# cipherflow-fhe/lattisense

Measured on AMD Instinct MI355X. Metric: ckks_hmult_relin_rescale_throughput, higher is better.
Workload: dtype u64

## Files before the change

lattisense_amd/csrc/emu_ntt.cpp:

```cpp
#define LSA_EMULATE 1
#include <cstddef>
#include <vector>
#include "ntt_plan.h"
#include "ntt_r16.h"
#include <array>
#include "tables.h"

template <int NT>
static void emu_block(const NttPassArgs& a, const NttBlockCtx& bc, u64* lds) {
    for (int t = 0; t < NT; t++) ntt_phase_load<true, NT>(a, bc, t, lds);
    int rho[4];
    const int np = ntt_split(a.mu, rho);
    if (!a.inverse) {
        int sig = 0;
        for (int i = 0; i < np; i++) {
            for (int t = 0; t < NT; t++) ntt_phase_sub_dyn<NT>(a, bc, t, lds, sig, rho[i]);
            sig += rho[i];
        }
    } else {
        int sig = a.mu;
        for (int i = np - 1; i >= 0; i--) {
            sig -= rho[i];
            for (int t = 0; t < NT; t++) ntt_phase_sub_dyn<NT>(a, bc, t, lds, sig, rho[i]);
        }
    }
    for (int t = 0; t < NT; t++) ntt_phase_store<true, NT>(a, bc, t, lds);
}

template <int PASS, int MU>
static void emu_block_r16(const NttPassArgs& a, const NttBlockCtx& bc, u64* lds) {
    std::vector<std::array<u64, 16>> regs(LSA_R16_THREADS);
    for (int phase = 0; phase < 3; phase++)
        for (int t = 0; t < LSA_R16_THREADS; t++) {
            u64(&v)[16] = *reinterpret_cast<u64(*)[16]>(regs[t].data());
            r16_phase<PASS, 3, MU>(a, bc, t, lds, phase, v);
        }
}

static void emu_block_r8x3(const NttPassArgs& a, const NttBlockCtx& bc, u64* lds) {
    std::vector<std::array<u64, 16>> regs(LSA_R16_THREADS);
    for (int phase = 0; phase < 4; phase++)
        for (int t = 0; t < LSA_R16_THREADS; t++) {
            u64(&v)[16] = *reinterpret_cast<u64(*)[16]>(regs[t].data());
            r8x3_phase<3>(a, bc, t, lds, phase, v);
        }
}

extern "C" int lsa_emu_ntt(int n, const u64* moduli, int nmod, u64* data, int batch, long long batch_stride, int rows,
                           const unsigned char* mod_of, int period, int inverse, int tau_max, int allow_fp64) {
    const int row_inner = (allow_fp64 >> 1) & 1;
    const bool r16 = (allow_fp64 >> 2) & 1;
    allow_fp64 &= 1;
    lsa::HostTables T;
    T.build(n, std::vector<u64>(moduli, moduli + nmod));
    NttPlan plan = make_ntt_plan(T.logn, tau_max);
    std::vector<u64> tw_i(T.psi.size());
    std::vector<double> tw_d(T.psi_d.size());
    for (int m = 0; m < nmod; m++) {
        const size_t o = (size_t)m * n;
        ntt_permute_twiddles(plan, T.logn, (inverse ? T.psiinv : T.psi).data() + 2 * o, tw_i.data() + 2 * o, 2, false);
        ntt_permute_twiddles(plan, T.logn, (inverse ? T.psiinv_d : T.psi_d).data() + o, tw_d.data() + o, 1, true);
    }
    NttPassArgs a{};
    a.src = data;
// ... 1 lines not shown
    a.src_stride = batch_stride;
    a.dst_stride = batch_stride;
    a.batch = batch;
    a.rows = rows;
    a.mods = T.mods.data();
    a.tw = tw_i.data();
    a.scale = T.scale.data();
    a.twd = tw_d.data();
    a.scaled = T.scale_d.data();
    a.allow_fp64 = allow_fp64;
    a.period = period;
    a.row0 = 0;
    a.row_step = 1;
    a.row_inner = row_inner;
    for (int i = 0; i < period; i++) a.mod_of[i] = mod_of[i];
    int launch_rows = 0;
    for (int r = 0; r < rows; r++)
        if (mod_of[r % period] != LSA_ROW_SKIP) a.row_tbl[launch_rows++] = (unsigned short)r;
    a.compact = 1;
    a.rows = launch_rows;
    for (int step = 0; step < plan.npass; step++) {
        int k = inverse ? plan.npass - 1 - step : step;
        ntt_fill_pass(a, plan, T.logn, k, inverse);
        a.fp_raw_out = plan.npass == 2 && step == 0;
        a.fp_raw_in = plan.npass == 2 && step == 1;
        std::vector<u64> lds(lds_words(a.tau));
        long long nblocks = (long long)batch * launch_rows * (1 << (a.logn - a.tau));
        for (long long bid = 0; bid < nblocks; bid++) {
            NttBlockCtx bc = ntt_decode_block(a, bid);
            if (bc.mod == LSA_ROW_SKIP) continue;
            if (r16 && ntt_r16_shape_ok(a, plan.npass)) {
                if (a.mu == 9) emu_block_r8x3(a, bc, lds.data());
                else if (a.lambda && a.mu == 8) emu_block_r16<0, 8>(a, bc, lds.data());
                else if (a.lambda) emu_block_r16<0, 7>(a, bc, lds.data());
                else if (a.mu == 8) emu_block_r16<1, 8>(a, bc, lds.data());
                else emu_block_r16<1, 7>(a, bc, lds.data());
            } else if (a.tau <= 12) emu_block<LSA_NTT_THREADS>(a, bc, lds.data());
            else if (a.tau == 13) emu_block<512>(a, bc, lds.data());
            else emu_block<1024>(a, bc, lds.data());
        }
    }
    return 0;
}
```

lattisense_amd/csrc/kernels.hip:

```cpp
#include <atomic>
#include <cstdlib>

#include "build_flags.h"
#include "lsa_internal.h"
#include "ntt_r16.h"

namespace lsa {

const char* kernels_build_flags() { return LSA_BUILD_FLAGS_TEXT; }

static constexpr int TPB = 256;

#ifndef LSA_NTT_WAVES
#define LSA_NTT_WAVES 4
#endif

#if defined(LSA_NTT_DIAG_STAMPS)
#define LSA_STAMP(k)                                                                               \
    do {                                                                                           \
        if (a.diag && threadIdx.x == 0 && blockIdx.x < 8192) a.diag[blockIdx.x * 8 + (k)] = __builtin_amdgcn_s_memtime(); \
    } while (0)
#else
#define LSA_STAMP(k) do { } while (0)
#endif
// ... 41 lines not shown
#if defined(LSA_NTT_STAGGER)
    {
        const int phase = blockIdx.x < 768 ? (int)(blockIdx.x >> 8) : 0;
        for (int i = 0; i < phase * LSA_NTT_STAGGER; i++) __builtin_amdgcn_s_sleep(100);
    }
#endif
#if defined(LSA_NTT_DIAG_COMPUTE_ONLY)
    for (int i = tid; i < (1 << a.tau); i += NT)
        lds[lds_addr(i)] = bc.fp ? d_to_bits((double)(i * 7 + 1)) : (u64)(i * 7 + 1);
    __syncthreads();
    ntt_butterfly_phases<NT>(a, bc, tid, lds);
    if (lds[lds_addr(tid)] == 0x123456789abcull) a.dst[bc.base_dst + tid] = 1;
    return;
#endif
    LSA_STAMP(0);
    ntt_phase_load<(FZ & 1) != 0, NT>(a, bc, tid, lds);
    if (TWL && tid < (1 << a.mu)) {
        u64* tw_l = lds + lds_words(a.tau);
        if (bc.fp) tw_l[tid] = twp.x;
        else {
            tw_l[2 * tid] = twp.x;
            tw_l[2 * tid + 1] = twp.y;
        }
    }
    LSA_STAMP(1);
    __syncthreads();
    LSA_STAMP(2);
#if defined(LSA_NTT_DIAG_COPY_ONLY)
    ntt_phase_store<(FZ & 2) != 0, NT, (FZ & 4) != 0, (FZ & 8) != 0>(a, bc, tid, lds);
    return;
#endif
// ... 42 lines not shown
    u64 v[16];
    r8x3_phase<FZ>(a, bc, tid, lds, 0, v);
    r16_sync<1>();
    r8x3_phase<FZ>(a, bc, tid, lds, 1, v);
    r16_sync<1>();
    r8x3_phase<FZ>(a, bc, tid, lds, 2, v);
    r16_sync<1>();
    r8x3_phase<FZ>(a, bc, tid, lds, 3, v);
}
static bool ntt_launch_r16(const NttPassArgs& a, int npass, bool fused, long long nblocks, hipStream_t s) {
    static const bool enabled = [] {
        const char* e = getenv("LSA_NTT_R16");
        return !(e && e[0] == '0');
    }();
    if (!enabled || !ntt_r16_shape_ok(a, npass)) return false;
    const bool pro = fused && a.fz_pro && a.s_lo == 0, epi = fused && a.fz_epi && a.final_reduce;
    const size_t lds_bytes = (size_t)LSA_R16_LDS_WORDS * sizeof(u64);
    const dim3 grid((unsigned)nblocks), block(LSA_R16_THREADS);
    if (epi && a.fz_epi == 3) {
        if (a.lambda) return false;
        if (a.mu == 9) {
            const char* e = getenv("LSA_NTT_R8X3");
            if (e && e[0] == '0') return false;
            hipLaunchKernelGGL((k_ntt_r8x3<4>), grid, block, lds_bytes, s, a);
        } else if (a.mu == 8) {
            hipLaunchKernelGGL((k_ntt_r16<1, 4, 8>), grid, block, lds_bytes, s, a);
        } else {
            hipLaunchKernelGGL((k_ntt_r16<1, 4, 7>), grid, block, lds_bytes, s, a);
        }
        LSA_HIP(hipGetLastError());
        return true;
    }
    if (epi && a.fz_epi == 4) {
// ... 73 lines not shown
    a.mu = MU;
    a.lambda = 0;
    a.tau = 12;
    a.inverse = 0;
    a.apply_scale = 0;
    a.final_reduce = 1;
    a.fp_raw_in = g.fp_raw_in;
    a.fp_raw_out = 0;
    a.mods = g.mods;
    a.tw = g.tw;
    a.twd = g.twd;
    a.scale = nullptr;
    a.scaled = nullptr;
    a.src = g.ext;
    a.fz_pro = a.fz_epi = 0;
    NttBlockCtx bc;
    bc.tile = tile;
    bc.mod = tl < g.L ? tl : g.nq + (tl - g.L);
    bc.fp = FP;
    bc.b = (int)b;
    bc.row = 0;
    bc.tw_l = nullptr;
    bc.base_dst = 0;
    const R16Limb L = r16_limb(a, bc);
    const int kj = tl < g.L ? tl : g.klvl + 1 + (tl - g.L);
    const int own_d = tl < g.L ? tl / g.np : -1;
    int k, i;
    r16_lane<1, MU>(tid, k, i);
    const unsigned G1 = r16_G1<1, MU>(bc, k), G2 = (G1 << 4) + ((unsigned)i << (MU <= 8 ? 8 - MU : 0));
    u64 acc0[16], acc1[16];
// ... 128 lines not shown
        int dev = 0;
        LSA_HIP(hipGetDevice(&dev));
        const unsigned long long bit = 1ull << (dev & 63);
        if (!(raised.load(std::memory_order_acquire) & bit)) {
            LSA_HIP(hipFuncSetAttribute(reinterpret_cast<const void*>(&k_ntt_pass<FZ, NT>), hipFuncAttributeMaxDynamicSharedMemorySize, 160 * 1024));
            raised.fetch_or(bit, std::memory_order_release);
        }
    }
    hipLaunchKernelGGL((k_ntt_pass<FZ, NT>), dim3((unsigned)nblocks), dim3(NT), lds_bytes, s, a);
    LSA_HIP(hipGetLastError());
}

template <int NT>
static void ntt_launch_pass(const NttPassArgs& a, bool fused, long long nblocks, size_t lds_bytes, hipStream_t s) {
    LSA_REQUIRE((1 << a.tau) <= 2 * LSA_NTT_STAGE_PAIRS * NT, "ntt: tile larger than the staging registers");
    const bool pro = fused && a.fz_pro && a.s_lo == 0, epi = fused && a.fz_epi && a.final_reduce;
    if (epi && a.fz_epi == 3) {
        ntt_launch_variant<4, NT>(a, nblocks, lds_bytes, s);
        return;
    }
    if (epi && a.fz_epi == 4) {
        ntt_launch_variant<8, NT>(a, nblocks, lds_bytes, s);
        return;
    }
    switch ((pro ? 1 : 0) | (epi ? 2 : 0)) {
        case 0: ntt_launch_variant<0, NT>(a, nblocks, lds_bytes, s); break;
        case 1: ntt_launch_variant<1, NT>(a, nblocks, lds_bytes, s); break;
        case 2: ntt_launch_variant<2, NT>(a, nblocks, lds_bytes, s); break;
        default: ntt_launch_variant<3, NT>(a, nblocks, lds_bytes, s); break;
    }
}
// ... 4 lines not shown
}

void launch_ntt(Context& c, const u64* src, u64* dst, int batch, long long src_stride, long long dst_stride, int rows,
                const RowMap& rm, bool inverse, hipStream_t s, const NttFusion* fz, int passes) {
    if (batch <= 0 || rows <= 0) return;
    LSA_REQUIRE(rm.period >= 1 && rm.period <= LSA_MAX_PERIOD, "ntt: bad row-map period");
    NttPassArgs a{};
    a.batch = batch;
    a.rows = rows;
    a.mods = c.d_mods;
    a.scale = c.d_scale;
    a.diag = c.ntt_diag;
    a.scaled = c.d_scale_d;
    a.allow_fp64 = c.fp64_ntt;
    if (fz) {
        LSA_REQUIRE(!inverse, "fused tails exist for forward transforms only");
        a.fz_epi = fz->epi;
        a.fz_pro = fz->pro;
        a.fz_limbs = fz->limbs;
        a.fz_base_polys = fz->base_polys;
        a.fz_ql_mod = fz->ql_mod;
        a.fz_a = fz->a;
        a.fz_a_stride = fz->a_stride;
        a.fz_a_rpp = fz->a_rpp;
        a.fz_base = fz->base;
        a.fz_base_stride = fz->base_stride;
        a.fz_base_rpp = fz->base_rpp;
        a.fz_k = fz->k;
        a.fz_out = fz->out;
        a.fz_out_stride = fz->out_stride;
        a.fz_out_rpp = fz->out_rpp;
        a.fz_last = fz->last;
        a.fz_last_stride = fz->last_stride;
        a.fz_last_rpp = fz->last_rpp;
        a.fz_k2 = fz->k2;
        a.fz_scatter = fz->scatter;
        LSA_REQUIRE(fz->epi != 2 || fz->k2, "merged tail needs its second factor");
        LSA_REQUIRE(!fz->scatter || fz->epi, "a scattered store needs an epilogue");
        LSA_REQUIRE(fz->epi != 3 || (!fz->pro && !fz->scatter && fz->a && fz->out), "pt_mul epilogue: plaintext and output, nothing else");
        LSA_REQUIRE(fz->epi != 4 || (!fz->pro && !fz->k2 && fz->scatter && fz->a && fz->k && fz->out && fz->pt),
                    "rotate-and-MAC epilogue: ModDown operands, index map, plaintext and output");
        LSA_REQUIRE(fz->epi != 4 || (fz->base_polys <= 1 && fz->limbs == rm.period), "rotate-and-MAC epilogue: base on poly 0, one row per limb");
        a.fz_pt = fz->pt;
        a.fz_pt_stride = fz->pt_stride;
        a.fz_accum = fz->accumulate ? 1 : 0;
    }
    a.period = rm.period;
    a.row0 = rm.row0;
    a.row_step = rm.row_step;
    for (int i = 0; i < rm.period; i++) {
        LSA_REQUIRE(rm.mod_of[i] == LSA_ROW_SKIP || rm.mod_of[i] < c.nmod, "ntt: modulus index out of range");
        a.mod_of[i] = rm.mod_of[i];
    }
    int active_rows = 0;
    for (int r = 0; r < rows; r++) active_rows += rm.mod_of[(rm.row0 + r * rm.row_step) % rm.period] != LSA_ROW_SKIP;
    if (active_rows == 0) return;
    int launch_rows = rows;
    a.compact = 0;
    if (active_rows <= LSA_MAX_PERIOD && rm.row0 + (rows - 1) * rm.row_step < 65536) {
        a.compact = 1;
// ... 4 lines not shown
        }
        launch_rows = active_rows;
    }
    a.rows = launch_rows;
    bool wide = c.plan_wide.npass < c.plan.npass && c.wide_mode != 0;
    if (wide && c.wide_mode == 2) {
        bool all_fp = c.fp64_ntt != 0;
        for (int r = 0; r < rows && all_fp; r++) {
            const unsigned char m = rm.mod_of[(rm.row0 + r * rm.row_step) % rm.period];
            if (m != LSA_ROW_SKIP && (c.T.mods[m].q >> LSA_FP64_MAX_BITS) != 0) all_fp = false;
        }
        const long long limbs = (long long)active_rows * batch;
        wide = !fz && (c.logn == 13 ? limbs >= 1024 : (all_fp && limbs >= 512));
    }
    if (passes != 3) wide = false;
    const NttPlan& plan = wide ? c.plan_wide : c.plan;
    a.tw = wide ? (inverse ? c.d_psiinv_w : c.d_psi_w) : (inverse ? c.d_psiinv : c.d_psi);
    a.twd = wide ? (inverse ? c.d_psiinv_d_w : c.d_psi_d_w) : (inverse ? c.d_psiinv_d : c.d_psi_d);
    {
        bool any_fp = false, any_int = false;
        for (int r = 0; r < rows; r++) {
            const unsigned char m = rm.mod_of[(rm.row0 + r * rm.row_step) % rm.period];
            if (m == LSA_ROW_SKIP) continue;
            const bool fp = c.fp_engine(m);
            any_fp |= fp;
            any_int |= !fp;
        }
        a.row_inner = any_fp && any_int;
    }
    int chunk = batch;
// ... 3 lines not shown
    }
    for (int b0 = 0; b0 < batch; b0 += chunk) {
        const int nb = std::min(chunk, batch - b0);
        a.batch = nb;
        if (fz && fz->epi == 3) {
            a.fz_a = fz->a + (long long)b0 * fz->a_stride;
            a.fz_base = fz->base ? fz->base + (long long)b0 * fz->base_stride : nullptr;
            a.fz_out = fz->out + (long long)b0 * fz->out_stride;
        }
        if (fz && fz->epi == 4) {
            a.fz_a = fz->a + (long long)b0 * fz->a_stride;
            a.fz_base = fz->base ? fz->base + (long long)b0 * fz->base_stride : nullptr;
            a.fz_pt = fz->pt + (long long)b0 * fz->pt_stride;
            a.fz_out = fz->out + (long long)b0 * fz->out_stride;
        }
        for (int step = 0; step < plan.npass; step++) {
            if (plan.npass == 2 && !((passes >> step) & 1)) continue;
            const int k = inverse ? plan.npass - 1 - step : step;
            ntt_fill_pass(a, plan, c.logn, k, inverse ? 1 : 0);
            a.fp_raw_out = plan.npass == 2 && step == 0 && c.fp_raw;
            a.fp_raw_in = plan.npass == 2 && step == 1 && c.fp_raw;
            a.src = (step == 0 ? src + (long long)b0 * src_stride : dst + (long long)b0 * dst_stride);
            a.src_stride = step == 0 ? src_stride : dst_stride;
            a.dst = dst + (long long)b0 * dst_stride;
            a.dst_stride = dst_stride;
            a.total_tiles = (long long)nb * launch_rows * (1 << (a.logn - a.tau));
            const long long nblocks = a.total_tiles;
            LSA_REQUIRE(nblocks < (1LL << 31), "ntt: grid too large");
            const size_t lds_bytes = (size_t)lds_words(a.tau) * sizeof(u64);
            ProfScope ps(c, PROF_NTT, 16.0 * c.n * active_rows * nb / plan.npass, s);
            if (ntt_launch_r16(a, plan.npass, fz != nullptr, nblocks, s)) continue;
            if (a.tau <= 12) ntt_launch_pass<LSA_NTT_THREADS>(a, fz != nullptr, nblocks, lds_bytes, s);
            else if (a.tau == 13) ntt_launch_pass<512>(a, fz != nullptr, nblocks, lds_bytes, s);
            else ntt_launch_pass<1024>(a, fz != nullptr, nblocks, lds_bytes, s);
        }
    }
}

struct EwArgs {
    const u64* a;
    const u64* b;
    const u64* acc;
    u64* out;
    long long sa, sb, so, sacc;
    const ModDev* mods;
// ... 400 lines not shown
    g.pb = (long long)(b_rpp ? b_rpp : limbs) << c.logn;
    g.a = a;
    g.b = b;
    g.d = d;
    g.sa = sa;
    g.sb = sb;
    g.sd = sd;
    g.mods = c.d_mods;
    g.limbs = limbs;
    g.logn = c.logn;
    LSA_REQUIRE(rm.period == limbs && limbs <= LSA_MAX_PERIOD, "tensor: row map must cover the limbs");
    int period;
    fill_rowmap(g.mod_of, period, rm, c.nmod);
    ProfScope ps(c, PROF_TENSOR, 7.0 * 8 * c.n * limbs * batch, s);
    hipLaunchKernelGGL(k_tensor, ew_grid(c, limbs, batch), dim3(TPB), 0, s, g);
    LSA_HIP(hipGetLastError());
}

__global__ __launch_bounds__(TPB) void k_tensor_d2(TensorArgs g) {
    const int chunks = (1 << g.logn) / (2 * TPB);
    const int limb = blockIdx.x / chunks;
    const int x = ((blockIdx.x % chunks) * TPB + threadIdx.x) * 2;
    const ModDev m = g.mods[limb];
    const long long b = blockIdx.y;
    const long long off = ((long long)limb << g.logn) + x;
    const ulonglong2 a1 = ld2(g.a + b * g.sa + g.pa + off), b1 = ld2(g.b + b * g.sb + g.pb + off);
    st2(g.d + b * g.sd + off, mont_mul(a1.x, mont_mul_lazy(b1.x, m.r2, m.q, m.qinv), m.q, m.qinv),
        mont_mul(a1.y, mont_mul_lazy(b1.y, m.r2, m.q, m.qinv), m.q, m.qinv));
}

void launch_tensor_d2(Context& c, const u64* a, const u64* b, u64* d2, int batch, long long sa, long long sb, long long sd,
                      int limbs, hipStream_t s, int a_rpp, int b_rpp) {
    if (batch <= 0) return;
    TensorArgs g{};
    LSA_REQUIRE((a_rpp == 0 || a_rpp >= limbs) && (b_rpp == 0 || b_rpp >= limbs), "tensor: rows per polynomial below the limb count");
    LSA_REQUIRE(limbs <= c.nq, "tensor: Q limbs only");
    g.pa = (long long)(a_rpp ? a_rpp : limbs) << c.logn;
    g.pb = (long long)(b_rpp ? b_rpp : limbs) << c.logn;
    g.a = a;
    g.b = b;
    g.d = d2;
    g.sa = sa;
    g.sb = sb;
    g.sd = sd;
    g.mods = c.d_mods;
    g.limbs = limbs;
    g.logn = c.logn;
    ProfScope ps(c, PROF_TENSOR, 3.0 * 8 * c.n * limbs * batch, s);
    hipLaunchKernelGGL(k_tensor_d2, ew_grid(c, limbs, batch), dim3(TPB), 0, s, g);
    LSA_HIP(hipGetLastError());
}

struct BaseConvArgs {
    const BaseConvConsts* k;
    const ModDev* mods;
    const u64* src;
    u64* dst;
    long long ssrc, sdst;
    int logn;
    BaseConvRows rows;
    const u64* sub;
    long long ssub;
    int sub_row[LSA_BC_MAX_SRC];
};
// ... 1188 lines not shown
```

lattisense_amd/csrc/lsa_internal.h:

```cpp
#pragma once
#include <hip/hip_runtime.h>
#include <cstdint>
#include <map>
#include <memory>
#include <mutex>
#include <stdexcept>
#include <string>
#include <vector>

#include "../../include/lattisense_amd.h"
#include "ntt_plan.h"
#include "tables.h"

namespace lsa {

struct Error : std::runtime_error {
    int code;
    Error(int c, const std::string& m) : std::runtime_error(m), code(c) {}
};

void set_last_error(const std::string& m);

#define LSA_HIP(expr)                                                                                     \
    do {                                                                                                  \
// ... 174 lines not shown
    const u64* base = nullptr;
    long long base_stride = 0;
    int base_rpp = 0;
    const u64* k = nullptr;
    u64* out = nullptr;
    long long out_stride = 0;
    int out_rpp = 0;
    const u64* last = nullptr;
    long long last_stride = 0;
    int last_rpp = 1;
    const u64* k2 = nullptr;
    const u32* scatter = nullptr;
    const u64* pt = nullptr;
    long long pt_stride = 0;
    bool accumulate = false;
};
void launch_ntt(Context& c, const u64* src, u64* dst, int batch, long long src_stride, long long dst_stride, int rows,
                const RowMap& rm, bool inverse, hipStream_t s, const NttFusion* fz = nullptr, int passes = 3);

enum EwOp { EW_ADD = 0, EW_SUB = 1, EW_NEG = 2, EW_MUL = 3 };
void launch_elementwise(Context& c, EwOp op, const u64* a, const u64* b, u64* out, int batch, long long sa,
                        long long sb, long long so, int rows, const RowMap& rm, hipStream_t s);
void launch_muladd(Context& c, EwOp op, const u64* a, const u64* b, const u64* acc, long long sacc, u64* out, int batch,
                   long long sa, long long sb, long long so, int rows, const RowMap& rm, hipStream_t s);
#define LSA_MAC_MAX_TERMS 16
#define LSA_MACM_MAX 8
void launch_mac_plain(Context& c, int terms, const u64* const* ct, const long long* sct, const u64* const* pt,
                      const long long* spt, const u64* partial, long long spartial, u64* out, long long so, int batch,
                      int polys, int limbs, const RowMap& rm, hipStream_t s);
void launch_mac_plain_multi(Context& c, int nb, const u64* const* ct, const long long* sct, int ng, const u64* const* pt,
                            u64* const* out, long long so, int batch, int polys, int limbs, const RowMap& rm, hipStream_t s);
void launch_mont_muladd(Context& c, const u64* a, long long sa, const u64* pt, long long spt, const u64* acc, long long sacc,
                        u64* out, long long so, int batch, int polys, int limbs, const RowMap& rm, hipStream_t s);
void launch_lift_ringt(Context& c, int mode, int level, const u64* pt, long long spt, u64* out, long long sout, int batch,
                       hipStream_t s);
void launch_tensor(Context& c, const u64* a, const u64* b, u64* d, int batch, long long sa, long long sb, long long sd,
                   int limbs, const RowMap& rm, hipStream_t s, int a_rpp = 0, int b_rpp = 0);
void launch_tensor_d2(Context& c, const u64* a, const u64* b, u64* d2, int batch, long long sa, long long sb, long long sd,
                      int limbs, hipStream_t s, int a_rpp = 0, int b_rpp = 0);
struct TensorFold {
    const u64* a;
    const u64* b;
    long long sa, sb;
    long long pa, pb;
};
struct BaseConvRows {
    int src_row[LSA_BC_MAX_SRC];
    int dst_row[LSA_BC_MAX_DST];
};
void launch_baseconv(Context& c, const BaseConvPlan* k, const BaseConvRows& rows, const u64* src, u64* dst, int batch,
                     long long ssrc, long long sdst, hipStream_t s, const u64* sub = nullptr, long long ssub = 0,
                     const int* sub_row = nullptr);
void launch_ks_mac(Context& c, int level, const u64* cx, long long scx, const u64* ext, long long sext,
                   const Key& key, u64* acc, long long sacc, int batch, hipStream_t s, bool unfused_only = false,
// ... 113 lines not shown
```

lattisense_amd/csrc/ntt_core.h:

```cpp
#pragma once
#include "modarith.h"

#ifndef LSA_NTT_THREADS
#define LSA_NTT_THREADS 256
#endif
#define LSA_MAX_PERIOD 192
#if defined(LSA_EMULATE)
#include <cstdio>
#include <cstdlib>
#define LSA_EMU_CHECK(c) do { if (!(c)) { std::fprintf(stderr, "ntt replay: range invariant violated: %s (%s:%d)\n", #c, __FILE__, __LINE__); std::abort(); } } while (0)
#else
#define LSA_EMU_CHECK(c) do { } while (0)
#endif
#define LSA_ROW_SKIP 0xFF
#define LSA_FP64_MAX_BITS 47
#ifndef LSA_NTT_MAX_RHO
#define LSA_NTT_MAX_RHO 4
#endif

struct NttPassArgs {
    const u64* src;
    u64* dst;
    long long src_stride;
    long long dst_stride;
// ... 19 lines not shown
    int fz_epi, fz_pro, fz_limbs, fz_base_polys, fz_ql_mod;
    int fz_a_rpp, fz_base_rpp, fz_out_rpp, fz_last_rpp;
    const u64* fz_a;
    const u64* fz_base;
    const u64* fz_k;
    const u64* fz_k2;
    u64* fz_out;
    const unsigned* fz_scatter;
    const u64* fz_last;
    long long fz_a_stride, fz_base_stride, fz_out_stride, fz_last_stride;
    unsigned long long* diag;
    unsigned char mod_of[LSA_MAX_PERIOD];
    const u64* fz_pt;
    long long fz_pt_stride;
    int fz_accum;
};

LSA_HD int lds_addr(int l) { return l + (l >> 4); }
LSA_HD int lds_words(int tau) { return (1 << tau) + (1 << (tau - 4)) + 16; }

LSA_HD long long ntt_tw_u_int(int s, int j, int k) {
#if defined(LSA_NTT_TW_NATURAL)
    return k;
#else
    return (long long)k << (s - j);
#endif
}
LSA_HD unsigned ntt_tw_v_int(int j, unsigned G) {
#if defined(LSA_NTT_TW_NATURAL)
    return G << j;
// ... 183 lines not shown
        return d_to_bits(f.add ? u52_to_double(v) + r : r);
    }
    if (f.head) {
        const u64 c = add_mod(t, f.h, f.ql);
        const u64 lift = sub_mod(f.near ? csub(c, f.mi.q) : reduce_u64(c, f.mi), f.hq, f.mi.q);
        v = f.add ? add_mod(v, lift, f.mi.q) : lift;
    }
    if (f.fp && !f.raw) v = d_to_bits(u52_to_double(v));
    return v;
}
template <bool FZ>
LSA_HD NttLoadFix ntt_make_load_fix(const NttPassArgs& a, const NttBlockCtx& bc, const u64*& g, const u64*& gl) {
    g = a.src + bc.base_src;
    gl = g;
    NttLoadFix f;
    f.head = FZ && a.fz_pro && a.s_lo == 0;
    f.add = f.head && a.fz_pro == 2;
    f.fp = bc.fp != 0;
    f.raw = f.fp && a.fp_raw_in;
    f.mi = a.mods[bc.mod];
    f.ql = f.h = f.hq = 0;
    f.hd = f.qld = 0.0;
    f.near = f.fp_lift = false;
    if (f.head) {
        gl = a.fz_last + (long long)bc.b * a.fz_last_stride + ((long long)(bc.row / a.fz_limbs) * a.fz_last_rpp << a.logn);
        if (!f.add) g = gl;
        f.ql = a.mods[a.fz_ql_mod].q;
        f.h = (f.ql - 1) >> 1;
        f.hq = reduce_u64(f.h, f.mi);
        f.near = f.ql <= 2 * f.mi.q;
        f.fp_lift = f.fp && (f.ql >> 48) == 0;
        f.hd = (double)f.h;
        f.qld = (double)f.ql;
    }
    return f;
}
template <bool FZ, int NT>
LSA_HD void ntt_phase_load(const NttPassArgs& a, const NttBlockCtx& bc, int tid, u64* lds) {
    const u64* g;
    const u64* gl;
    const int half = 1 << (a.tau - 1);
    const NttLoadFix f = ntt_make_load_fix<FZ>(a, bc, g, gl);
    const NttTileMap tm = ntt_tile_map(a, bc.tile);
    if (half == LSA_NTT_STAGE_PAIRS * NT && !f.add) {
        NttLoadFix f1 = f;
        f1.add = false;
        u64 st[2 * LSA_NTT_STAGE_PAIRS];
#pragma unroll
        for (int p = 0; p < LSA_NTT_STAGE_PAIRS; p++) {
            const int x = ntt_tile_index(tm, 2 * (tid + p * NT));
            ntt_load_data_pair(g + x, st[2 * p], st[2 * p + 1]);
        }
#pragma unroll
        for (int p = 0; p < LSA_NTT_STAGE_PAIRS; p++) {
            const int l = 2 * (tid + p * NT);
            lds[lds_addr(l)] = ntt_load_fix(f1, st[2 * p], st[2 * p]);
// ... 645 lines not shown
```

lattisense_amd/csrc/ntt_r16.h:

```cpp
#pragma once
#include "ntt_core.h"

#define LSA_R16_THREADS 256
#define LSA_R16_LDS_WORDS (272 * 16)

LSA_HD bool ntt_r16_shape_ok(const NttPassArgs& a, int npass) {
    if (npass != 2 || a.tau != 12) return false;
    if (a.mu == 9) return a.s_lo == a.logn - 9 && a.lambda == 0;
    if (a.mu != 8 && a.mu != 7) return false;
    return (a.s_lo == 0 && a.lambda == 12 - a.mu) || (a.s_lo == a.logn - a.mu && a.lambda == 0);
}

template <int PASS, int MU>
LSA_HD int r16_lds(int k, int i) {
    const int p = i + (i >> 4);
    return PASS == 0 ? (p << (12 - MU)) + k : k * ((1 << MU) + (1 << (MU - 4))) + p;
}
template <int PASS, int MU>
LSA_HD long long r16_x(const NttPassArgs& a, int tile, int k, int i) {
    return PASS == 0 ? ((long long)tile << (12 - MU)) + ((long long)i << (a.logn - MU)) + k : ((long long)tile << 12) + (k << MU) + i;
}
template <int MU, int IMAGE>
LSA_HD int r16_pt(int i, int e) {
    return IMAGE == 0 ? i + (e << (MU - 4)) : 16 * i + e;
// ... 173 lines not shown
}
template <int PASS, int IMAGE, int MU>
LSA_HD void r16_lds_get(int tid, const u64* lds, u64 (&v)[16]) {
    int k, i;
    r16_lane<PASS, MU>(tid, k, i);
#pragma unroll
    for (int e = 0; e < 16; e++) v[e] = lds[r16_lds<PASS, MU>(k, r16_pt<MU, IMAGE>(i, e))];
}
template <int MU>
LSA_HD void r16_pair_pos(int tid, int m, int& k, int& i) {
    const int wave = tid >> 6, lane = tid & 63;
    const int c = 2 * (lane + 64 * m);
    k = (wave << (10 - MU)) + (c >> MU);
    i = c & ((1 << MU) - 1);
}
template <bool FZ, int MU>
LSA_HD void r16_load_coalesced(const NttPassArgs& a, const NttBlockCtx& bc, int tid, u64* lds) {
    const u64* g;
    const u64* gl;
    NttLoadFix f = ntt_make_load_fix<FZ>(a, bc, g, gl);
    f.add = false;
    u64 st[16];
#pragma unroll
    for (int m = 0; m < 8; m++) {
        int k, i;
        r16_pair_pos<MU>(tid, m, k, i);
        ntt_load_data_pair(g + r16_x<1, MU>(a, bc.tile, k, i), st[2 * m], st[2 * m + 1]);
    }
#pragma unroll
    for (int m = 0; m < 8; m++) {
        int k, i;
        r16_pair_pos<MU>(tid, m, k, i);
// ... 186 lines not shown
        if (phase == 0) {
            r16_load_direct<PASS, (FZ & 1) != 0, 0, MU>(a, bc, tid, v);
            r16_group<PASS, 0, MU>(v, a, bc, L, G1);
            r16_lds_put<PASS, 0, MU>(tid, lds, v);
        } else if (phase == 1) {
            r16_lds_get<PASS, 1, MU>(tid, lds, v);
            r16_group<PASS, 1, MU>(v, a, bc, L, G2);
            if (PASS == 0) r16_store_direct<PASS, (FZ & 2) != 0, 1, MU>(a, bc, tid, v);
            else r16_lds_put<PASS, 1, MU>(tid, lds, v);
        } else if (PASS == 1) {
            r16_store_coalesced<(FZ & 2) != 0, MU, (FZ & 4) != 0, (FZ & 8) != 0>(a, bc, tid, lds);
        }
    } else {
        if (phase == 0) {
            if (PASS == 0) r16_load_direct<PASS, false, 1, MU>(a, bc, tid, v);
            else r16_load_coalesced<false, MU>(a, bc, tid, lds);
        } else if (phase == 1) {
            if (PASS == 1) r16_lds_get<PASS, 1, MU>(tid, lds, v);
            r16_group<PASS, 1, MU>(v, a, bc, L, G2);
            r16_lds_put<PASS, 1, MU>(tid, lds, v);
        } else {
            r16_lds_get<PASS, 0, MU>(tid, lds, v);
            r16_group<PASS, 0, MU>(v, a, bc, L, G1);
            r16_store_direct<PASS, false, 0, MU>(a, bc, tid, v);
        }
    }
}

template <int IMAGE>
LSA_HD int r8x3_pt(int i, int E) {
    if (IMAGE == 0) return i + (E << 5);
// ... 48 lines not shown
            r8x3_group<0>(v, a, bc, L, G1, i);
            r8x3_put<0>(k, i, lds, v);
        } else if (phase == 1) {
            r8x3_get<1>(k, i, lds, v);
            r8x3_group<1>(v, a, bc, L, G1, i);
            r8x3_put<1>(k, i, lds, v);
        } else if (phase == 2) {
            r8x3_get<2>(k, i, lds, v);
            r8x3_group<2>(v, a, bc, L, G1, i);
            r8x3_put<2>(k, i, lds, v);
        } else {
            r16_store_coalesced<(FZ & 2) != 0, 9, (FZ & 4) != 0, (FZ & 8) != 0>(a, bc, tid, lds);
        }
    } else {
        if (phase == 0) {
            r16_load_coalesced<false, 9>(a, bc, tid, lds);
        } else if (phase == 1) {
            r8x3_get<2>(k, i, lds, v);
            r8x3_group<2>(v, a, bc, L, G1, i);
            r8x3_put<2>(k, i, lds, v);
        } else if (phase == 2) {
            r8x3_get<1>(k, i, lds, v);
            r8x3_group<1>(v, a, bc, L, G1, i);
            r8x3_put<1>(k, i, lds, v);
        } else {
            r8x3_get<0>(k, i, lds, v);
            r8x3_group<0>(v, a, bc, L, G1, i);
            r16_store_direct<1, false, 0, 9>(a, bc, tid, v);
        }
    }
}
// ... 157 lines not shown
```

lattisense_amd/csrc/ops.hip:

```cpp
#include "lsa_internal.h"

namespace lsa {

static RowMap rm_seq(int count, int first = 0) {
    RowMap r;
    LSA_REQUIRE(count >= 1 && count <= LSA_MAX_PERIOD, "row map too long");
    r.period = count;
    for (int i = 0; i < count; i++) r.mod_of[i] = (unsigned char)(first + i);
    return r;
}

static int ceil_div(int a, int b) { return (a + b - 1) / b; }

struct KsRescale {
    u64* out;
    long long sout;
};

struct RotMacTerm {
    const u64* pt;
    long long spt;
    bool accumulate;
};

// ... 152 lines not shown
        const long long N = c.n;
        L = level + 1;
        T = L + c.np;
        beta = ceil_div(L, c.np);
        fused = key && ks_fuse_mac(c, level, *key);
        s_cxi = (long long)L * N;
        s_ext = (long long)beta * T * N;
        s_acc = 2LL * T * N;
        s_conv = 2LL * L * N;
        cxi = ws;
        ext = cxi + (size_t)nb * s_cxi;
        acc = ext + (size_t)nb * s_ext;
        conv = acc + (size_t)nb * s_acc;
    }

    void decompose(const u64* cx, long long scx, const u64* cx_coef = nullptr, long long s_coef = 0) {
        const long long N = c.n;
        const int np = c.np;
        if (!cx_coef) launch_ntt(c, cx, cxi, nb, scx, s_cxi, L, rm_seq(L), true, s);
        const u64* conv_src = cx_coef ? cx_coef : cxi;
        const long long s_src = cx_coef ? s_coef : s_cxi;
        for (int d = 0; d < beta; d++) {
            const int d0 = d * np, d1 = std::min(d0 + np, L);
            std::vector<int> src, dst;
            BaseConvRows rows{};
            for (int i = d0; i < d1; i++) {
                rows.src_row[i - d0] = i;
                src.push_back(i);
            }
            for (int tl = 0; tl < T; tl++) {
                if (tl >= d0 && tl < d1) continue;
                rows.dst_row[dst.size()] = d * T + tl;
                dst.push_back(c.qp_mod(L, tl));
            }
// ... 273 lines not shown
void ckks_mult_relin_rescale(Context& c, int level, const u64* a, const u64* b, const Key& rlk, u64* out, int batch,
                             long long sa, long long sb, long long so, hipStream_t s) {
    ckks_mult_relin_rescale_rpp(c, level, a, b, rlk, out, batch, sa, sb, so, s, 0, 0);
}
static bool hmult_fold_on() {
    const char* e = std::getenv("LSA_HMULT_FOLD");
    return !(e && e[0] == '0');
}

void ckks_mult_relin_rescale_rpp(Context& c, int level, const u64* a, const u64* b, const Key& rlk, u64* out, int batch,
                                 long long sa, long long sb, long long so, hipStream_t s, int a_rpp, int b_rpp) {
    LSA_REQUIRE(level >= 1, "mult+relin+rescale needs level >= 1");
    const long long N = c.n;
    const int L = level + 1;
    const bool fold = c.fuse_tails && hmult_fold_on();
    const size_t r_d3 = (fold ? 1 : 3) * (size_t)L, r_r2 = 2 * (size_t)L;
    const size_t r_shared = std::max(KsTile::rows(c, level), rescale_ws_rows(level, 2));
    const long long sd = (long long)r_d3 * N, sr = 2LL * L * N;
    for_tiles(c, r_d3 + r_r2 + r_shared, batch, s, [&](int nb, int b0, u64* ws, int tb, hipStream_t st) {
        u64* d3 = ws;
        u64* r2 = d3 + r_d3 * N * tb;
        u64* sub = r2 + r_r2 * N * tb;
        if (fold) {
            const u64* ta = a + (size_t)b0 * sa;
            const u64* bt = b + (size_t)b0 * sb;
            launch_tensor_d2(c, ta, bt, d3, nb, sa, sb, sd, L, st, a_rpp, b_rpp);
            const TensorFold tf{ta, bt, sa, sb, (long long)(a_rpp ? a_rpp : L) * N, (long long)(b_rpp ? b_rpp : L) * N};
            KsTile t(c, level, nb, sub, st, &rlk);
            t.decompose(d3, sd);
            t.mac(d3, sd, rlk, &tf);
            t.moddown({.p = r2, .sp = sr, .form = KsOut::RESCALE, .rs = {out + (size_t)b0 * so, so}});
            return;
        }
        launch_tensor(c, a + (size_t)b0 * sa, b + (size_t)b0 * sb, d3, nb, sa, sb, sd, L, rm_seq(L), st, a_rpp, b_rpp);
        KsOut o{.p = r2, .sp = sr, .base = d3, .sbase = sd, .base_rpp = L, .base_polys = 2};
        if (c.fuse_tails) {
            o.form = KsOut::RESCALE;
            o.rs = {out + (size_t)b0 * so, so};
            key_switch(c, level, d3 + 2LL * L * N, sd, rlk, o, nb, sub, st);
            return;
        }
        key_switch(c, level, d3 + 2LL * L * N, sd, rlk, o, nb, sub, st);
        rescale(c, level, 2, r2, sr, out + (size_t)b0 * so, so, nb, true, sub, st);
    });
}
// ... 358 lines not shown
```

Baseline: 13700.

## Fuse d2 tensor product into the inverse NTT prologue of key switching

Removes the separate k_tensor_d2 kernel that wrote the d2 = a1*b1 product to a workspace. The inverse NTT's first pass now loads a1 and b1 directly and multiplies them modularly before the butterflies, in both the generic and radix-16/r8x3 paths. The MAC then reads the coefficient-domain buffer instead of the evaluation-domain d2. This saves one global write and read of L limbs plus a launch, shrinks the per-tile workspace, and adds a product-prologue template variant.

```diff
diff --git a/lattisense_amd/csrc/emu_ntt.cpp b/lattisense_amd/csrc/emu_ntt.cpp
--- a/lattisense_amd/csrc/emu_ntt.cpp
+++ b/lattisense_amd/csrc/emu_ntt.cpp
@@ -8,7 +8,7 @@
 
 template <int NT>
 static void emu_block(const NttPassArgs& a, const NttBlockCtx& bc, u64* lds) {
-    for (int t = 0; t < NT; t++) ntt_phase_load<true, NT>(a, bc, t, lds);
+    for (int t = 0; t < NT; t++) ntt_phase_load<true, NT, true>(a, bc, t, lds);
     int rho[4];
     const int np = ntt_split(a.mu, rho);
     if (!a.inverse) {
@@ -33,7 +33,7 @@
     for (int phase = 0; phase < 3; phase++)
         for (int t = 0; t < LSA_R16_THREADS; t++) {
             u64(&v)[16] = *reinterpret_cast<u64(*)[16]>(regs[t].data());
-            r16_phase<PASS, 3, MU>(a, bc, t, lds, phase, v);
+            r16_phase<PASS, 3 | 16, MU>(a, bc, t, lds, phase, v);
         }
 }
 
@@ -42,12 +42,12 @@
     for (int phase = 0; phase < 4; phase++)
         for (int t = 0; t < LSA_R16_THREADS; t++) {
             u64(&v)[16] = *reinterpret_cast<u64(*)[16]>(regs[t].data());
-            r8x3_phase<3>(a, bc, t, lds, phase, v);
+            r8x3_phase<3 | 16>(a, bc, t, lds, phase, v);
         }
 }
 
-extern "C" int lsa_emu_ntt(int n, const u64* moduli, int nmod, u64* data, int batch, long long batch_stride, int rows,
-                           const unsigned char* mod_of, int period, int inverse, int tau_max, int allow_fp64) {
+static int emu_ntt(int n, const u64* moduli, int nmod, u64* data, int batch, long long batch_stride, int rows,
+                   const unsigned char* mod_of, int period, int inverse, int tau_max, int allow_fp64, const u64* pa, const u64* pb) {
     const int row_inner = (allow_fp64 >> 1) & 1;
     const bool r16 = (allow_fp64 >> 2) & 1;
     allow_fp64 &= 1;
@@ -79,6 +79,14 @@
     a.row_step = 1;
     a.row_inner = row_inner;
     for (int i = 0; i < period; i++) a.mod_of[i] = mod_of[i];
+    if (pa) {
+        a.fz_pro = 3;
+        a.fz_limbs = rows;
+        a.fz_a = pa;
+        a.fz_b = pb;
+        a.fz_a_stride = a.fz_b_stride = batch_stride;
+        a.fz_a_rpp = a.fz_b_rpp = rows;
+    }
     int launch_rows = 0;
     for (int r = 0; r < rows; r++)
         if (mod_of[r % period] != LSA_ROW_SKIP) a.row_tbl[launch_rows++] = (unsigned short)r;
@@ -87,6 +95,7 @@
     for (int step = 0; step < plan.npass; step++) {
         int k = inverse ? plan.npass - 1 - step : step;
         ntt_fill_pass(a, plan, T.logn, k, inverse);
+        a.fz_first = step == 0;
         a.fp_raw_out = plan.npass == 2 && step == 0;
         a.fp_raw_in = plan.npass == 2 && step == 1;
         std::vector<u64> lds(lds_words(a.tau));
@@ -107,3 +116,15 @@
     }
     return 0;
 }
+
+extern "C" int lsa_emu_ntt(int n, const u64* moduli, int nmod, u64* data, int batch, long long batch_stride, int rows,
+                           const unsigned char* mod_of, int period, int inverse, int tau_max, int allow_fp64) {
+    return emu_ntt(n, moduli, nmod, data, batch, batch_stride, rows, mod_of, period, inverse, tau_max, allow_fp64, nullptr, nullptr);
+}
+
+extern "C" int lsa_emu_intt_prod(int n, const u64* moduli, int nmod, const u64* pa, const u64* pb, u64* out, int batch,
+                                 long long batch_stride, int rows, const unsigned char* mod_of, int period, int tau_max,
+                                 int allow_fp64) {
+    if (!pa || !pb) return -1;
+    return emu_ntt(n, moduli, nmod, out, batch, batch_stride, rows, mod_of, period, 1, tau_max, allow_fp64, pa, pb);
+}
diff --git a/lattisense_amd/csrc/kernels.hip b/lattisense_amd/csrc/kernels.hip
--- a/lattisense_amd/csrc/kernels.hip
+++ b/lattisense_amd/csrc/kernels.hip
@@ -79,7 +79,7 @@
     return;
 #endif
     LSA_STAMP(0);
-    ntt_phase_load<(FZ & 1) != 0, NT>(a, bc, tid, lds);
+    ntt_phase_load<(FZ & 1) != 0, NT, (FZ & 16) != 0>(a, bc, tid, lds);
     if (TWL && tid < (1 << a.mu)) {
         u64* tw_l = lds + lds_words(a.tau);
         if (bc.fp) tw_l[tid] = twp.x;
@@ -152,9 +152,23 @@
         return !(e && e[0] == '0');
     }();
     if (!enabled || !ntt_r16_shape_ok(a, npass)) return false;
-    const bool pro = fused && a.fz_pro && a.s_lo == 0, epi = fused && a.fz_epi && a.final_reduce;
+    const bool pro = fused && a.fz_pro && a.fz_first, epi = fused && a.fz_epi && a.final_reduce;
     const size_t lds_bytes = (size_t)LSA_R16_LDS_WORDS * sizeof(u64);
     const dim3 grid((unsigned)nblocks), block(LSA_R16_THREADS);
+    if (pro && a.fz_pro == 3) {
+        if (a.lambda || !a.inverse) return false;
+        if (a.mu == 9) {
+            const char* e = getenv("LSA_NTT_R8X3");
+            if (e && e[0] == '0') return false;
+            hipLaunchKernelGGL((k_ntt_r8x3<16>), grid, block, lds_bytes, s, a);
+        } else if (a.mu == 8) {
+            hipLaunchKernelGGL((k_ntt_r16<1, 16, 8>), grid, block, lds_bytes, s, a);
+        } else {
+            hipLaunchKernelGGL((k_ntt_r16<1, 16, 7>), grid, block, lds_bytes, s, a);
+        }
+        LSA_HIP(hipGetLastError());
+        return true;
+    }
     if (epi && a.fz_epi == 3) {
         if (a.lambda) return false;
         if (a.mu == 9) {
@@ -258,6 +272,7 @@
     a.scaled = nullptr;
     a.src = g.ext;
     a.fz_pro = a.fz_epi = 0;
+    a.fz_first = 0;
     NttBlockCtx bc;
     bc.tile = tile;
     bc.mod = tl < g.L ? tl : g.nq + (tl - g.L);
@@ -416,7 +431,12 @@
 template <int NT>
 static void ntt_launch_pass(const NttPassArgs& a, bool fused, long long nblocks, size_t lds_bytes, hipStream_t s) {
     LSA_REQUIRE((1 << a.tau) <= 2 * LSA_NTT_STAGE_PAIRS * NT, "ntt: tile larger than the staging registers");
-    const bool pro = fused && a.fz_pro && a.s_lo == 0, epi = fused && a.fz_epi && a.final_reduce;
+    const bool pro = fused && a.fz_pro && a.fz_first, epi = fused && a.fz_epi && a.final_reduce;
+    if (pro && a.fz_pro == 3) {
+        if constexpr (NT == LSA_NTT_THREADS) ntt_launch_variant<16, NT>(a, nblocks, lds_bytes, s);
+        else LSA_REQUIRE(false, "ntt: the product prologue needs a tile of at most 4096 points");
+        return;
+    }
     if (epi && a.fz_epi == 3) {
         ntt_launch_variant<4, NT>(a, nblocks, lds_bytes, s);
         return;
@@ -451,7 +471,9 @@
     a.scaled = c.d_scale_d;
     a.allow_fp64 = c.fp64_ntt;
     if (fz) {
-        LSA_REQUIRE(!inverse, "fused tails exist for forward transforms only");
+        LSA_REQUIRE(!inverse || (fz->pro == 3 && !fz->epi), "inverse transforms take the product prologue only");
+        LSA_REQUIRE(fz->pro != 3 || (inverse && !fz->epi && fz->a && fz->b && fz->limbs >= 1 && (passes & 1)),
+                    "product prologue: an inverse transform from its first pass, two operands, no epilogue");
         a.fz_epi = fz->epi;
         a.fz_pro = fz->pro;
         a.fz_limbs = fz->limbs;
@@ -481,6 +503,9 @@
         a.fz_pt = fz->pt;
         a.fz_pt_stride = fz->pt_stride;
         a.fz_accum = fz->accumulate ? 1 : 0;
+        a.fz_b = fz->b;
+        a.fz_b_stride = fz->b_stride;
+        a.fz_b_rpp = fz->b_rpp;
     }
     a.period = rm.period;
     a.row0 = rm.row0;
@@ -515,6 +540,7 @@
         wide = !fz && (c.logn == 13 ? limbs >= 1024 : (all_fp && limbs >= 512));
     }
     if (passes != 3) wide = false;
+    if (fz && fz->pro == 3) wide = false;
     const NttPlan& plan = wide ? c.plan_wide : c.plan;
     a.tw = wide ? (inverse ? c.d_psiinv_w : c.d_psi_w) : (inverse ? c.d_psiinv : c.d_psi);
     a.twd = wide ? (inverse ? c.d_psiinv_d_w : c.d_psi_d_w) : (inverse ? c.d_psiinv_d : c.d_psi_d);
@@ -548,12 +574,20 @@
             a.fz_pt = fz->pt + (long long)b0 * fz->pt_stride;
             a.fz_out = fz->out + (long long)b0 * fz->out_stride;
         }
+        if (fz && fz->pro == 3) {
+            a.fz_a = fz->a + (long long)b0 * fz->a_stride;
+            a.fz_b = fz->b + (long long)b0 * fz->b_stride;
+        }
+        bool first = true;
         for (int step = 0; step < plan.npass; step++) {
             if (plan.npass == 2 && !((passes >> step) & 1)) continue;
+            a.fz_first = first ? 1 : 0;
+            first = false;
             const int k = inverse ? plan.npass - 1 - step : step;
             ntt_fill_pass(a, plan, c.logn, k, inverse ? 1 : 0);
             a.fp_raw_out = plan.npass == 2 && step == 0 && c.fp_raw;
             a.fp_raw_in = plan.npass == 2 && step == 1 && c.fp_raw;
+            LSA_REQUIRE(!(a.fz_first && a.fz_pro && a.fp_raw_in), "ntt: a fused prologue reads canonical inputs, never a raw hand-off");
             a.src = (step == 0 ? src + (long long)b0 * src_stride : dst + (long long)b0 * dst_stride);
             a.src_stride = step == 0 ? src_stride : dst_stride;
             a.dst = dst + (long long)b0 * dst_stride;
@@ -562,7 +596,8 @@
             const long long nblocks = a.total_tiles;
             LSA_REQUIRE(nblocks < (1LL << 31), "ntt: grid too large");
             const size_t lds_bytes = (size_t)lds_words(a.tau) * sizeof(u64);
-            ProfScope ps(c, PROF_NTT, 16.0 * c.n * active_rows * nb / plan.npass, s);
+            const double pro_bytes = fz && fz->pro == 3 && a.fz_first ? 8.0 * c.n * active_rows * nb : 0.0;
+            ProfScope ps(c, PROF_NTT, 16.0 * c.n * active_rows * nb / plan.npass + pro_bytes, s);
             if (ntt_launch_r16(a, plan.npass, fz != nullptr, nblocks, s)) continue;
             if (a.tau <= 12) ntt_launch_pass<LSA_NTT_THREADS>(a, fz != nullptr, nblocks, lds_bytes, s);
             else if (a.tau == 13) ntt_launch_pass<512>(a, fz != nullptr, nblocks, lds_bytes, s);
@@ -993,40 +1028,6 @@
     fill_rowmap(g.mod_of, period, rm, c.nmod);
     ProfScope ps(c, PROF_TENSOR, 7.0 * 8 * c.n * limbs * batch, s);
     hipLaunchKernelGGL(k_tensor, ew_grid(c, limbs, batch), dim3(TPB), 0, s, g);
-    LSA_HIP(hipGetLastError());
-}
-
-__global__ __launch_bounds__(TPB) void k_tensor_d2(TensorArgs g) {
-    const int chunks = (1 << g.logn) / (2 * TPB);
-    const int limb = blockIdx.x / chunks;
-    const int x = ((blockIdx.x % chunks) * TPB + threadIdx.x) * 2;
-    const ModDev m = g.mods[limb];
-    const long long b = blockIdx.y;
-    const long long off = ((long long)limb << g.logn) + x;
-    const ulonglong2 a1 = ld2(g.a + b * g.sa + g.pa + off), b1 = ld2(g.b + b * g.sb + g.pb + off);
-    st2(g.d + b * g.sd + off, mont_mul(a1.x, mont_mul_lazy(b1.x, m.r2, m.q, m.qinv), m.q, m.qinv),
-        mont_mul(a1.y, mont_mul_lazy(b1.y, m.r2, m.q, m.qinv), m.q, m.qinv));
-}
-
-void launch_tensor_d2(Context& c, const u64* a, const u64* b, u64* d2, int batch, long long sa, long long sb, long long sd,
-                      int limbs, hipStream_t s, int a_rpp, int b_rpp) {
-    if (batch <= 0) return;
-    TensorArgs g{};
-    LSA_REQUIRE((a_rpp == 0 || a_rpp >= limbs) && (b_rpp == 0 || b_rpp >= limbs), "tensor: rows per polynomial below the limb count");
-    LSA_REQUIRE(limbs <= c.nq, "tensor: Q limbs only");
-    g.pa = (long long)(a_rpp ? a_rpp : limbs) << c.logn;
-    g.pb = (long long)(b_rpp ? b_rpp : limbs) << c.logn;
-    g.a = a;
-    g.b = b;
-    g.d = d2;
-    g.sa = sa;
-    g.sb = sb;
-    g.sd = sd;
-    g.mods = c.d_mods;
-    g.limbs = limbs;
-    g.logn = c.logn;
-    ProfScope ps(c, PROF_TENSOR, 3.0 * 8 * c.n * limbs * batch, s);
-    hipLaunchKernelGGL(k_tensor_d2, ew_grid(c, limbs, batch), dim3(TPB), 0, s, g);
     LSA_HIP(hipGetLastError());
 }
 
diff --git a/lattisense_amd/csrc/lsa_internal.h b/lattisense_amd/csrc/lsa_internal.h
--- a/lattisense_amd/csrc/lsa_internal.h
+++ b/lattisense_amd/csrc/lsa_internal.h
@@ -212,6 +212,9 @@
     const u64* pt = nullptr;
     long long pt_stride = 0;
     bool accumulate = false;
+    const u64* b = nullptr;
+    long long b_stride = 0;
+    int b_rpp = 0;
 };
 void launch_ntt(Context& c, const u64* src, u64* dst, int batch, long long src_stride, long long dst_stride, int rows,
                 const RowMap& rm, bool inverse, hipStream_t s, const NttFusion* fz = nullptr, int passes = 3);
@@ -234,8 +237,6 @@
                        hipStream_t s);
 void launch_tensor(Context& c, const u64* a, const u64* b, u64* d, int batch, long long sa, long long sb, long long sd,
                    int limbs, const RowMap& rm, hipStream_t s, int a_rpp = 0, int b_rpp = 0);
-void launch_tensor_d2(Context& c, const u64* a, const u64* b, u64* d2, int batch, long long sa, long long sb, long long sd,
-                      int limbs, hipStream_t s, int a_rpp = 0, int b_rpp = 0);
 struct TensorFold {
     const u64* a;
     const u64* b;
diff --git a/lattisense_amd/csrc/ntt_core.h b/lattisense_amd/csrc/ntt_core.h
--- a/lattisense_amd/csrc/ntt_core.h
+++ b/lattisense_amd/csrc/ntt_core.h
@@ -57,6 +57,10 @@
     const u64* fz_pt;
     long long fz_pt_stride;
     int fz_accum;
+    const u64* fz_b;
+    long long fz_b_stride;
+    int fz_b_rpp;
+    int fz_first;
 };
 
 LSA_HD int lds_addr(int l) { return l + (l >> 4); }
@@ -270,10 +274,11 @@
     g = a.src + bc.base_src;
     gl = g;
     NttLoadFix f;
-    f.head = FZ && a.fz_pro && a.s_lo == 0;
+    f.head = FZ && (a.fz_pro == 1 || a.fz_pro == 2) && a.fz_first;
     f.add = f.head && a.fz_pro == 2;
     f.fp = bc.fp != 0;
     f.raw = f.fp && a.fp_raw_in;
+    LSA_EMU_CHECK(!(a.fz_pro && a.fz_first && a.fp_raw_in));
     f.mi = a.mods[bc.mod];
     f.ql = f.h = f.hq = 0;
     f.hd = f.qld = 0.0;
@@ -291,11 +296,65 @@
     }
     return f;
 }
-template <bool FZ, int NT>
+struct NttProdFix {
+    const u64* pa;
+    const u64* pb;
+    ModDev mi;
+    double qd, qinvd;
+    bool fp;
+};
+LSA_HD NttProdFix ntt_make_prod_fix(const NttPassArgs& a, const NttBlockCtx& bc) {
+    const int poly = bc.row / a.fz_limbs, limb = bc.row % a.fz_limbs;
+    NttProdFix p;
+    p.pa = a.fz_a + (long long)bc.b * a.fz_a_stride + (((long long)poly * a.fz_a_rpp + limb) << a.logn);
+    p.pb = a.fz_b + (long long)bc.b * a.fz_b_stride + (((long long)poly * a.fz_b_rpp + limb) << a.logn);
+    p.mi = a.mods[bc.mod];
+    p.fp = bc.fp != 0;
+    p.qd = (double)p.mi.q;
+    p.qinvd = 1.0 / p.qd;
+    LSA_EMU_CHECK(!a.fp_raw_in);
+    return p;
+}
+LSA_HD u64 ntt_prod_fix(const NttProdFix& p, u64 x, u64 y) {
+    LSA_EMU_CHECK(x < p.mi.q && y < p.mi.q);
+    if (p.fp) return d_to_bits(fp_reduce(fp_modmul(u52_to_double(x), u52_to_double(y), p.qd, p.qinvd), p.qd, p.qinvd));
+    return mont_mul(x, mont_mul_lazy(y, p.mi.r2, p.mi.q, p.mi.qinv), p.mi.q, p.mi.qinv);
+}
+template <bool FZ, int NT, bool PR = false>
 LSA_HD void ntt_phase_load(const NttPassArgs& a, const NttBlockCtx& bc, int tid, u64* lds) {
     const u64* g;
     const u64* gl;
     const int half = 1 << (a.tau - 1);
+    if (PR && a.fz_pro == 3 && a.fz_first) {
+        const NttProdFix pf = ntt_make_prod_fix(a, bc);
+        const NttTileMap tm = ntt_tile_map(a, bc.tile);
+        if (half == LSA_NTT_STAGE_PAIRS * NT) {
+            constexpr int CH = LSA_NTT_STAGE_PAIRS / LSA_NTT_HEAD_ROUNDS;
+#pragma unroll 1
+            for (int p0 = 0; p0 < LSA_NTT_STAGE_PAIRS; p0 += CH) {
+                u64 sa[2 * CH], sb[2 * CH];
+#pragma unroll
+                for (int p = 0; p < CH; p++) {
+                    const int x = ntt_tile_index(tm, 2 * (tid + (p0 + p) * NT));
+                    ntt_load_data_pair(pf.pa + x, sa[2 * p], sa[2 * p + 1]);
+                    ntt_load_data_pair(pf.pb + x, sb[2 * p], sb[2 * p + 1]);
+                }
+#pragma unroll
+                for (int p = 0; p < CH; p++) {
+                    const int l = 2 * (tid + (p0 + p) * NT);
+                    lds[lds_addr(l)] = ntt_prod_fix(pf, sa[2 * p], sb[2 * p]);
+                    lds[lds_addr(l + 1)] = ntt_prod_fix(pf, sa[2 * p + 1], sb[2 * p + 1]);
+                }
+            }
+            return;
+        }
+        for (int i = tid; i < half; i += NT) {
+            const int x = ntt_tile_index(tm, 2 * i);
+            lds[lds_addr(2 * i)] = ntt_prod_fix(pf, pf.pa[x], pf.pb[x]);
+            lds[lds_addr(2 * i + 1)] = ntt_prod_fix(pf, pf.pa[x + 1], pf.pb[x + 1]);
+        }
+        return;
+    }
     const NttLoadFix f = ntt_make_load_fix<FZ>(a, bc, g, gl);
     const NttTileMap tm = ntt_tile_map(a, bc.tile);
     if (half == LSA_NTT_STAGE_PAIRS * NT && !f.add) {
diff --git a/lattisense_amd/csrc/ntt_r16.h b/lattisense_amd/csrc/ntt_r16.h
--- a/lattisense_amd/csrc/ntt_r16.h
+++ b/lattisense_amd/csrc/ntt_r16.h
@@ -211,8 +211,36 @@
     k = (wave << (10 - MU)) + (c >> MU);
     i = c & ((1 << MU) - 1);
 }
-template <bool FZ, int MU>
+template <bool FZ, int MU, bool PR = false>
 LSA_HD void r16_load_coalesced(const NttPassArgs& a, const NttBlockCtx& bc, int tid, u64* lds) {
+    if (PR && a.fz_pro == 3 && a.fz_first) {
+        const NttProdFix pf = ntt_make_prod_fix(a, bc);
+        u64 sa[16], sb[16];
+#pragma unroll
+        for (int m = 0; m < 8; m++) {
+            int k, i;
+            r16_pair_pos<MU>(tid, m, k, i);
+            const long long x = r16_x<1, MU>(a, bc.tile, k, i);
+            ntt_load_data_pair(pf.pa + x, sa[2 * m], sa[2 * m + 1]);
+            ntt_load_data_pair(pf.pb + x, sb[2 * m], sb[2 * m + 1]);
+        }
+        if (pf.fp) {
+#pragma unroll
+            for (int j = 0; j < 16; j++)
+                sa[j] = d_to_bits(fp_reduce(fp_modmul(u52_to_double(sa[j]), u52_to_double(sb[j]), pf.qd, pf.qinvd), pf.qd, pf.qinvd));
+        } else {
+#pragma unroll
+            for (int j = 0; j < 16; j++) sa[j] = ntt_prod_fix(pf, sa[j], sb[j]);
+        }
+#pragma unroll
+        for (int m = 0; m < 8; m++) {
+            int k, i;
+            r16_pair_pos<MU>(tid, m, k, i);
+            lds[r16_lds<1, MU>(k, i)] = sa[2 * m];
+            lds[r16_lds<1, MU>(k, i + 1)] = sa[2 * m + 1];
+        }
+        return;
+    }
     const u64* g;
     const u64* gl;
     NttLoadFix f = ntt_make_load_fix<FZ>(a, bc, g, gl);
@@ -429,7 +457,7 @@
     } else {
         if (phase == 0) {
             if (PASS == 0) r16_load_direct<PASS, false, 1, MU>(a, bc, tid, v);
-            else r16_load_coalesced<false, MU>(a, bc, tid, lds);
+            else r16_load_coalesced<false, MU, (FZ & 16) != 0>(a, bc, tid, lds);
         } else if (phase == 1) {
             if (PASS == 1) r16_lds_get<PASS, 1, MU>(tid, lds, v);
             r16_group<PASS, 1, MU>(v, a, bc, L, G2);
@@ -508,7 +536,7 @@
         }
     } else {
         if (phase == 0) {
-            r16_load_coalesced<false, 9>(a, bc, tid, lds);
+            r16_load_coalesced<false, 9, (FZ & 16) != 0>(a, bc, tid, lds);
         } else if (phase == 1) {
             r8x3_get<2>(k, i, lds, v);
             r8x3_group<2>(v, a, bc, L, G1, i);
diff --git a/lattisense_amd/csrc/ops.hip b/lattisense_amd/csrc/ops.hip
--- a/lattisense_amd/csrc/ops.hip
+++ b/lattisense_amd/csrc/ops.hip
@@ -190,10 +190,24 @@
         conv = acc + (size_t)nb * s_acc;
     }
 
-    void decompose(const u64* cx, long long scx, const u64* cx_coef = nullptr, long long s_coef = 0) {
+    void decompose(const u64* cx, long long scx, const u64* cx_coef = nullptr, long long s_coef = 0, const TensorFold* prod = nullptr) {
         const long long N = c.n;
         const int np = c.np;
-        if (!cx_coef) launch_ntt(c, cx, cxi, nb, scx, s_cxi, L, rm_seq(L), true, s);
+        if (prod) {
+            LSA_REQUIRE(!cx_coef, "key switch: a product source has no coefficient-domain copy");
+            NttFusion fz;
+            fz.pro = 3;
+            fz.limbs = L;
+            fz.a = prod->a + prod->pa;
+            fz.a_stride = prod->sa;
+            fz.a_rpp = (int)(prod->pa >> c.logn);
+            fz.b = prod->b + prod->pb;
+            fz.b_stride = prod->sb;
+            fz.b_rpp = (int)(prod->pb >> c.logn);
+            launch_ntt(c, cxi, cxi, nb, s_cxi, s_cxi, L, rm_seq(L), true, s, &fz);
+        } else if (!cx_coef) {
+            launch_ntt(c, cx, cxi, nb, scx, s_cxi, L, rm_seq(L), true, s);
+        }
         const u64* conv_src = cx_coef ? cx_coef : cxi;
         const long long s_src = cx_coef ? s_coef : s_cxi;
         for (int d = 0; d < beta; d++) {
@@ -497,7 +511,7 @@
     const long long N = c.n;
     const int L = level + 1;
     const bool fold = c.fuse_tails && hmult_fold_on();
-    const size_t r_d3 = (fold ? 1 : 3) * (size_t)L, r_r2 = 2 * (size_t)L;
+    const size_t r_d3 = (fold ? 0 : 3) * (size_t)L, r_r2 = 2 * (size_t)L;
     const size_t r_shared = std::max(KsTile::rows(c, level), rescale_ws_rows(level, 2));
     const long long sd = (long long)r_d3 * N, sr = 2LL * L * N;
     for_tiles(c, r_d3 + r_r2 + r_shared, batch, s, [&](int nb, int b0, u64* ws, int tb, hipStream_t st) {
@@ -507,11 +521,11 @@
         if (fold) {
             const u64* ta = a + (size_t)b0 * sa;
             const u64* bt = b + (size_t)b0 * sb;
-            launch_tensor_d2(c, ta, bt, d3, nb, sa, sb, sd, L, st, a_rpp, b_rpp);
+            LSA_REQUIRE((a_rpp == 0 || a_rpp >= L) && (b_rpp == 0 || b_rpp >= L), "tensor: rows per polynomial below the limb count");
             const TensorFold tf{ta, bt, sa, sb, (long long)(a_rpp ? a_rpp : L) * N, (long long)(b_rpp ? b_rpp : L) * N};
             KsTile t(c, level, nb, sub, st, &rlk);
-            t.decompose(d3, sd);
-            t.mac(d3, sd, rlk, &tf);
+            t.decompose(nullptr, 0, nullptr, 0, &tf);
+            t.mac(t.cxi, t.s_cxi, rlk, &tf);
             t.moddown({.p = r2, .sp = sr, .form = KsOut::RESCALE, .rs = {out + (size_t)b0 * so, so}});
             return;
         }
```

After: 14190, median of 6. +3.6%, better.
